# ZwwWayne/mmMOT

Hardware: AMD Instinct MI355X
Metric: frame-pairs/sec (fusion+affinity fwd) at N_det=64; affinity L∞ vs CPU ref (higher is better)
Workload: dtype f16x3

## Files before the change

include/mmmot_hip.h:

```cpp
#ifndef MMMOT_HIP_H
#define MMMOT_HIP_H

#include <stddef.h>
#include <stdint.h>

#ifdef __cplusplus
extern "C" {
#endif

#define MMMOT_OK 0
#define MMMOT_EINVAL (-1)

#define MMMOT_ACT_NONE 0
#define MMMOT_ACT_RELU 1
#define MMMOT_ACT_SIGMOID 2

#define MMMOT_A_PLAIN 0
#define MMMOT_A_NORM_RELU 1
#define MMMOT_A_PAIR 2

#define MMMOT_PAIR_MULTIPLY 0
#define MMMOT_PAIR_MINUS_ABS 1
#define MMMOT_PAIR_MINUS 2

// ... 101 lines not shown

int mmmot_gn_finalize(const float* part, const int* grp_tile0, const int* grp_ntiles,
                      const int* grp_count, const int* tile_nrows, int G, int ldp, int C, int NG,
                      const float* gamma, const float* beta, float eps,
                      float* sc, float* sh, void* stream);

int mmmot_segment_mean(const float* X, int ldx, int C,
                       const int* seg_start, const int* seg_count, const int* seg_stride,
                       const int* seg_group, const int* seg_div, int nseg,
                       const float* sc, const float* sh, int ldsc, int relu,
                       float* out, int ldo,
                       int hl16 ,
                       void* stream);

int mmmot_rowdot(const float* X, int ldx, int K, const float* w, float b,
                 const float* sc, const float* sh, int ldsc,
                 const int* tile_row0, const int* tile_nrows, const int* tile_group, int T,
                 int act, int use_thr, float thr,
                 float* out, const int* omap, void* stream);

int mmmot_row_layernorm(const float* X, int ldx, int C, const float* gamma, const float* beta,
                        float eps, int relu, float* Y, int ldy, int R, void* stream);

int mmmot_skippool_head(const float* P, int ldp, int C, int C4, const float* g0, const float* b0, const float* w1,
                        const float* c1, const float* g2, const float* b2, const float* w4, const float* c4,
                        const float* g5, const float* b5, float eps, float* out, int ldo, int R, void* stream);
int mmmot_pointnet_layer1(const float* X, int K, const float* W, const float* bias,
                          float* Y, float* part,
                          const int* tile_row0, const int* tile_nrows, int T, void* stream);

int mmmot_pn_mlp64(const float* X, int ldx, const float* sc, const float* sh, int ldsc, const void* W16,
                   float oscale, const float* bias, float* Y, int ldy, float* part, const int* tile_row0,
                   const int* tile_nrows, const int* tile_group, int T, int N, void* stream);

int mmmot_affine_act(const float* X, int ldx, int C, const float* sc, const float* sh, int ldsc,
                     const int* tile_row0, const int* tile_nrows, const int* tile_group, int T,
                     int act, float* Y, int ldy, void* stream);

int mmmot_fusion_combine(int mode, const float* cat, const float* Y0, int ld0,
                         const float* Y1, int ld1,
                         const float* sc0, const float* sh0, const float* sc1, const float* sh1, int ldsc,
                         const int* tile_row0, const int* tile_nrows, const int* tile_group, int T,
                         float* F, int Lt, int C, void* stream);

int mmmot_softmax_pairs(const float* logits, float* out,
                        const int* grp_row0, const int* grp_N, const int* grp_M, int G,
                        int max_nm ,
                        int mode, void* stream);

int mmmot_points_count(const float* pts, int P, int F, const double* planes, int NB, int pad_empty,
                       int* cnt, int* split, void* stream);
int mmmot_points_scatter(const float* pts, int P, int F, const double* planes, int NB, const int* cnt,
                         const int* split, float* out, int Fo, void* stream);
int mmmot_points_count_batched(const float* pts, int F, int NS, int NPOLY, int NBLK, int cnt_total,
                               const double* planes, const int* blk_sweep, const int* blk_first,
                               const int* sweep_row0, const int* poly0, const int* filt, const int* cnt_off,
                               int pad_empty, int* cnt, int* split, void* stream);
int mmmot_points_scatter_batched(const float* pts, int F, int NS, int NPOLY, int NBLK, int cnt_total,
                                 const double* planes, const int* blk_sweep, const int* blk_first,
                                 const int* sweep_row0, const int* poly0, const int* filt, const int* cnt_off,
                                 const int* cnt, const int* split, float* out, int Fo, void* stream);

#define MMMOT_ALIGN_MAX_CHAIN 4
#define MMMOT_ALIGN_REC 80
int mmmot_align_points(const float* pts, int F, int Q, int NS, const int* seg_row0, const double* xf, int chain,
                       float* out, long out_row0, int ldo, void* stream);
// ... 148 lines not shown
```

mmmot_amd/_lib.py:

```python
import ctypes
import os
import subprocess
import threading

_HERE = os.path.dirname(os.path.abspath(__file__))
CSRC = os.path.join(_HERE, 'csrc')
LIB_PATH = os.environ.get('MMMOT_LIB_PATH', os.path.join(_HERE, 'libmmmot_hip.so'))
SOURCES = ['conv3x3.hip', 'hl16_format.hip', 'conv3x3_hl16_patch.hip', 'gemm_rows.hip', 'gemm_wide.hip',
           'gemm_ares.hip', 'gemm_wres.hip', 'gemm_wreg.hip', 'pn_mlp64.hip', 'gram.hip', 'points_gather.hip', 'crop_resize.hip', 'crop_augment.hip','small_kernels.hip', 'backward.hip', 'train.hip', 'train_vgg.hip', 'gemm_tn_f16.hip',
           'assign.hip', 'assign_chain.hip', 'track_ids.hip', 'clear_mot.hip', 'align_points.hip', 'labels.hip', 'adam_step.hip', 'dropout.hip']
HIPCC = os.environ.get('HIPCC', '/opt/rocm/bin/hipcc')
HIPFLAGS = ['--offload-arch=gfx950', '-O3', '-std=c++17', '-fPIC']

_lock = threading.Lock()
_lib = None

c_f = ctypes.c_void_p
c_i = ctypes.c_int


class GemmArgs(ctypes.Structure):
    _fields_ = [
        ('X', c_f), ('ldx', c_i),
        ('W', c_f),
# ... 54 lines not shown
    'mmmot_gram_rows': [c_f, c_i, c_i, c_f, c_f, c_i, c_f, c_f, c_f, c_i, c_f, c_f, c_f],
    'mmmot_set_gram128_variant': [c_i],
    'mmmot_gn_finalize_gram': [c_f, c_f, c_f, c_f, c_f, c_i, c_i, c_f, c_f, c_i, c_f, c_f, ctypes.c_float, c_f, c_f, c_f, c_f],
    'mmmot_gn_finalize_gram_dbias': [c_f, c_f, c_f, c_f, c_f, c_i, c_f, c_f, c_i, c_f, c_f, c_i, c_i, c_f, c_f, ctypes.c_float,
                                     c_f, c_f, c_f, c_f],
    'mmmot_gn_finalize': [c_f, c_f, c_f, c_f, c_f, c_i, c_i, c_i, c_i, c_f, c_f, ctypes.c_float, c_f, c_f, c_f],
    'mmmot_segment_mean': [c_f, c_i, c_i, c_f, c_f, c_f, c_f, c_f, c_i, c_f, c_f, c_i, c_i, c_f, c_i, c_i, c_f],
    'mmmot_conv3x3_bn_relu_hl16_patch': [c_f, c_f, c_f, c_f, c_i, c_i, c_i, c_i, c_i, c_i, c_f, c_f],
    'mmmot_conv1_fused_hl16': [c_f, c_f, c_f, ctypes.c_float, c_f, c_f, c_f, c_f, c_i, c_i, c_i, c_f],
    'mmmot_conv3x3_bn_relu_hq8': [c_f, c_f, c_f, c_f, c_i, c_i, c_i, c_i, c_i, c_i, c_f, c_f],
    'mmmot_conv1_fused_u8': [c_f, ctypes.c_float, ctypes.c_float, ctypes.c_float, ctypes.c_float, ctypes.c_float,
                             ctypes.c_float, c_f, c_f, ctypes.c_float, c_f, c_f, c_f, c_f, c_i, c_i, c_i, c_i, c_f],
    'mmmot_u8_normalize': [c_f, c_i, c_i, c_f, c_f, c_f],
    'mmmot_conv1_fused_hq8': [c_f, c_f, c_f, ctypes.c_float, c_f, c_f, c_f, c_f, c_i, c_i, c_i, c_f],
    'mmmot_conv3x3_first_hl16': [c_f, c_f, c_f, c_f, c_i, c_i, c_i, c_i, c_f],
    'mmmot_set_patch_grid_limit': [c_i],
    'mmmot_set_patch_min_block': [c_i],
    'mmmot_trunk_range_read': [ctypes.POINTER(ctypes.c_uint), c_i],
    'mmmot_trunk_range_bind': [c_f],
    'mmmot_hl16_pack': [c_f, c_f, ctypes.c_long, c_f],
    'mmmot_hl16_unpack': [c_f, c_f, ctypes.c_long, c_f],
    'mmmot_hl16_pack_pow2': [c_f, c_f, ctypes.c_long, c_f, c_i, c_f],
    'mmmot_pow2_oscale': [c_f, c_i, c_f, c_i, c_f, c_i, c_f],
    'mmmot_conv3x3_raw_hl16': [c_f, c_f, c_f, c_f, c_i, c_i, c_i, c_i, c_i, c_f, c_f],
    'mmmot_hq8_pack': [c_f, c_f, ctypes.c_long, c_f],
    'mmmot_hq8_unpack': [c_f, c_f, ctypes.c_long, c_f],
    'mmmot_rowdot': [c_f, c_i, c_i, c_f, ctypes.c_float, c_f, c_f, c_i, c_f, c_f, c_f, c_i, c_i, c_i,
                     ctypes.c_float, c_f, c_f, c_f],
    'mmmot_row_layernorm': [c_f, c_i, c_i, c_f, c_f, ctypes.c_float, c_i, c_f, c_i, c_i, c_f],
    'mmmot_skippool_head': [c_f, c_i, c_i, c_i, c_f, c_f, c_f, c_f, c_f, c_f, c_f, c_f, c_f, c_f, ctypes.c_float, c_f, c_i, c_i,
                            c_f],
    'mmmot_pointnet_layer1': [c_f, c_i, c_f, c_f, c_f, c_f, c_f, c_f, c_i, c_f],
    'mmmot_pn_mlp64': [c_f, c_i, c_f, c_f, c_i, c_f, ctypes.c_float, c_f, c_f, c_i, c_f, c_f, c_f, c_f, c_i, c_i, c_f],
    'mmmot_affine_act': [c_f, c_i, c_i, c_f, c_f, c_i, c_f, c_f, c_f, c_i, c_i, c_f, c_i, c_f],
    'mmmot_fusion_combine': [c_i, c_f, c_f, c_i, c_f, c_i, c_f, c_f, c_f, c_f, c_i, c_f, c_f, c_f, c_i, c_f,
                             c_i, c_i, c_f],
    'mmmot_softmax_pairs': [c_f, c_f, c_f, c_f, c_f, c_i, c_i, c_i, c_f],
    'mmmot_points_count': [c_f, c_i, c_i, c_f, c_i, c_i, c_f, c_f, c_f],
    'mmmot_points_scatter': [c_f, c_i, c_i, c_f, c_i, c_f, c_f, c_f, c_i, c_f],
    'mmmot_crop_resize_norm': [c_f, c_i, c_i, c_f, c_i, c_i, c_i, c_f, c_f, c_f, c_f, c_f],
    'mmmot_crop_augment': [c_f, c_f, c_i, c_i, c_f, c_f, c_f, c_f],
    'mmmot_points_count_batched': [c_f, c_i, c_i, c_i, c_i, c_i, c_f, c_f, c_f, c_f, c_f, c_f, c_f, c_i, c_f, c_f, c_f],
    'mmmot_points_scatter_batched': [c_f, c_i, c_i, c_i, c_i, c_i, c_f, c_f, c_f, c_f, c_f, c_f, c_f, c_f, c_f, c_f, c_i, c_f],
    'mmmot_align_points': [c_f, c_i, c_i, c_i, c_f, c_f, c_i, c_f, ctypes.c_long, c_i, c_f],
    'mmmot_selftest_mfma': [c_f, c_f, c_f, c_i, c_f],
    'mmmot_gn_bwd_partial': [c_f, c_i, c_f, c_i, c_i, c_f, c_f, c_i, c_f, c_f, c_i, c_f, c_f, c_f, c_i, c_f, c_f],
    'mmmot_gn_bwd_finalize': [c_f, c_f, c_i, c_i, c_i, c_f, c_f, c_f],
    'mmmot_gn_bwd_apply': [c_f, c_i, c_f, c_i, c_i, c_f, c_f, c_i, c_f, c_f, c_i, c_f, c_f, c_f, c_f, c_i, c_f, c_i, c_f],
    'mmmot_gemm_tn': [ctypes.POINTER(GemmTnArgs), c_f],
    'mmmot_gemm_tn_f16': [ctypes.POINTER(GemmTnArgs), c_f, c_f],
    'mmmot_absmax': [c_f, c_i, ctypes.c_long, c_i, c_f, c_f],
    'mmmot_pair_bwd': [c_f, c_i, c_f, c_i, c_f, c_i, c_i, c_f, c_f, c_f, c_f, c_f, c_f, c_f, c_i, c_i, c_i, c_f],
    'mmmot_pair_expand_bwd': [c_f, c_i, c_f, c_i, c_i, c_f, c_f, c_f, c_i, c_f, c_f, c_f, c_f, c_f],
    'mmmot_segment_argmax': [c_f, c_i, c_i, c_f, c_f, c_f, c_f, c_i, c_f, c_f, c_i, c_i, c_f, c_i, c_f],
    'mmmot_pair_expand_max_bwd': [c_f, c_i, c_f, c_i, c_f, c_i, c_i, c_f, c_f, c_f, c_i, c_f, c_f, c_f, c_f, c_f],
    'mmmot_rowdot_bwd': [c_f, c_i, c_i, c_f, ctypes.c_float, c_f, c_f, c_i, c_f, c_f, c_f, c_i, c_i, c_f, c_f, c_f, c_i,
                         c_f, c_i, c_f],
    'mmmot_softmax_pairs_bwd': [c_f, c_f, c_f, c_f, c_f, c_f, c_i, c_i, c_i, c_f],
    'mmmot_fusion_c_bwd': [c_f, c_f, c_i, c_f, c_i, c_f, c_f, c_f, c_f, c_i, c_f, c_f, c_f, c_i, c_f, c_f, c_i, c_f, c_f, c_i, c_f],
    'mmmot_add_rows': [c_f, c_i, c_f, c_i, c_f, c_i, ctypes.c_long, c_i, c_f],
    'mmmot_conv3x3_raw': [c_f, c_f, c_f, c_f, c_i, c_i, c_i, c_i, c_i, c_i, c_f],
    'mmmot_rows_stats': [c_f, c_i, c_i, c_f, c_f, c_i, c_f, c_f],
    'mmmot_bn_relu_pool': [c_f, c_i, c_f, c_f, c_i, c_i, c_i, c_i, c_f, c_f],
    'mmmot_maxpool_bwd': [c_f, c_i, c_f, c_f, c_f, c_i, c_i, c_i, c_f, c_f],
    'mmmot_conv3x3_wgrad': [c_f, c_f, c_i, c_i, c_i, c_i, c_i, c_i, c_f, c_f],
    'mmmot_conv3x3_wgrad_f16': [c_f, c_f, c_i, c_i, c_i, c_i, c_i, c_i, c_f, c_f, c_f],
# ... 93 lines not shown
```

mmmot_amd/csrc/pn_mlp64.hip:

```cpp
#include "common.h"

#define PM_K 64
#define PM_LDT 72

template <int NOUT>
__global__ __launch_bounds__(256) void pn_mlp64_kernel(const float* __restrict__ X, int ldx,
                                                       const float* __restrict__ sc, const float* __restrict__ sh,
                                                       int ldsc, const u32x4* __restrict__ W16, float oscale,
                                                       const float* __restrict__ bias, float* __restrict__ Y, int ldy,
                                                       float* __restrict__ part, const int* __restrict__ tile_row0,
                                                       const int* __restrict__ tile_nrows,
                                                       const int* __restrict__ tile_group, int T) {
  constexpr int NT = NOUT / 32;
  __shared__ __attribute__((aligned(16))) _Float16 Wh[NOUT * PM_LDT];
  __shared__ __attribute__((aligned(16))) _Float16 Wl[NOUT * PM_LDT];
  __shared__ __attribute__((aligned(16))) _Float16 Ah[MM_BM * PM_LDT];
  __shared__ __attribute__((aligned(16))) _Float16 Al[MM_BM * PM_LDT];
  __shared__ float red[2][4][NOUT];
  const int tid = threadIdx.x, lane = tid & 63, wave = tid >> 6;
  const int lr = lane & 31, kh = (lane >> 5) * 8;

  for (int idx = tid; idx < NOUT * 8; idx += 256) {
    const int n = idx >> 3, u = idx & 7;
    const u32x4 hi = W16[(long)idx * 2], lo = W16[(long)idx * 2 + 1];
// ... 77 lines not shown
          s1 += acc[nt][e];
          Y[(long)(row0 + wave * 32 + mm_acc_row(e, lane)) * ldy + nt * 32 + lr] = acc[nt][e];
        }
      }
      s1 = mm_xor32_sum(s1);
      if (lane < 32) red[0][wave][nt * 32 + lr] = s1;
    }
    __syncthreads();
    const float inv = 1.f / (float)nrows;
#pragma unroll
    for (int nt = 0; nt < NT; ++nt) {
      const int n = nt * 32 + lr;
      const float tot = red[0][0][n] + red[0][1][n] + red[0][2][n] + red[0][3][n];
      const float mu = tot * inv;
      float s2 = 0.f;
#pragma unroll
      for (int e = 0; e < 16; ++e) {
        const float d = acc[nt][e] - mu;
        if (valid[e]) s2 = fmaf(d, d, s2);
      }
      s2 = mm_xor32_sum(s2);
      if (lane < 32) red[1][wave][n] = s2;
      if (wave == 0 && lane < 32) part[((long)t * 2 + 0) * NOUT + n] = tot;
    }
    __syncthreads();
    if (wave == 0 && lane < 32) {
#pragma unroll
      for (int nt = 0; nt < NT; ++nt) {
        const int n = nt * 32 + lr;
        part[((long)t * 2 + 1) * NOUT + n] = red[1][0][n] + red[1][1][n] + red[1][2][n] + red[1][3][n];
      }
    }
  }
}

extern "C" int mmmot_pn_mlp64(const float* X, int ldx, const float* sc, const float* sh, int ldsc, const void* W16,
                              float oscale, const float* bias, float* Y, int ldy, float* part, const int* tile_row0,
                              const int* tile_nrows, const int* tile_group, int T, int N, void* stream) {
  if (!X || !sc || !sh || !W16 || !Y || !part || !tile_row0 || !tile_nrows || T <= 0) return MMMOT_EINVAL;
  if ((N != 64 && N != 128) || ldx % 4 != 0 || ldsc % 4 != 0 || ldy < N) return MMMOT_EINVAL;
  if (!mm_al16(X) || !mm_al16(sc) || !mm_al16(sh) || !mm_al16(W16)) return MMMOT_EINVAL;
  const int n_cu = mm_num_cu();
  if (n_cu <= 0) return MMMOT_EINVAL;
  const int grid = T < 2 * n_cu ? T : 2 * n_cu;
  hipStream_t s = (hipStream_t)stream;
  if (N == 64)
    hipLaunchKernelGGL(pn_mlp64_kernel<64>, dim3(grid), dim3(256), 0, s, X, ldx, sc, sh, ldsc, (const u32x4*)W16, oscale,
                       bias, Y, ldy, part, tile_row0, tile_nrows, tile_group, T);
  else
    hipLaunchKernelGGL(pn_mlp64_kernel<128>, dim3(grid), dim3(256), 0, s, X, ldx, sc, sh, ldsc, (const u32x4*)W16, oscale,
                       bias, Y, ldy, part, tile_row0, tile_nrows, tile_group, T);
  return mm_check(hipGetLastError());
}
```

mmmot_amd/engine.py:

```python
import contextlib
import itertools
import os
import threading

import numpy as np
import torch

from .ops import (ACT_NONE, ACT_RELU, ACT_SIGMOID, A_NORM_RELU, A_PAIR, A_PLAIN, FUSION_MODES, PAIR_OPS,
                  SOFTMAX_MODES)
from .range_guard import RangeGuard
from .tape import norm_layer

POOL_INPUT = {'f32': 0, 'hl16': 1, 'hq8': 2}
EPS = 1e-5
_SERIALS = itertools.count(1)


def check_crop_side(S):
    if S < 32 or S % 2 != 0:
        raise ValueError('crop side %d is not supported: the HIP VGG trunk needs an even side >= 32; resize the crops '
                         '(mmmot_amd.crops.crop_resize_normalize)' % S)


def check_crop_layout(dets):
# ... 2 lines not shown
            raise ValueError('uint8 crops must be [L,S,S,3] (HWC, the output of mmmot_amd.crops.crop_resize_u8), got %s'
                             % (tuple(dets.shape),))
        S = int(dets.shape[1])
    else:
        S = int(dets.shape[-1])
    check_crop_side(S)
    return S


class Engine:
    eps = EPS

    def __init__(self, packed, ops, fusion='A', affinity_op='multiply', softmax_mode='none',
                 neg_threshold=0.0, score_arch='branch_cls', end_mode='avg', trunk=None):
        trunk = trunk or os.environ.get('MMMOT_TRUNK', 'f16x3')
        if trunk not in ('f16x3', 'f16q8', 'f32'):
            raise ValueError("trunk must be 'f16x3' (fp16 matrix cores, 3-term split), 'f16q8' (fp16 main term + "
                             "fp8 correction terms, include/mmmot_hip.h hq8) or 'f32' (exact fp32 MFMA)")
        self.trunk = trunk
        self.serial = next(_SERIALS)
        self.trunk_requested = trunk
        self.guard = RangeGuard(self)
        self.range_events = []
        self.last_out_of_range_forward = None
        self.out_of_range_window = None
        self._busy = threading.Lock()
        self._last_stream = None
        self._head_start = None
        ql = os.environ.get('MMMOT_Q8_LAYERS', '4,5,6,7,8,9,10,11,12')
        self.q8_layers = None if ql == 'all' else set(int(v) for v in ql.split(',') if v)
        self.pn_fused = os.environ.get('MMMOT_PN_FUSED', '1') != '0'
        self.pn_gram = os.environ.get('MMMOT_PN_GRAM', '1') != '0'
        self.pn_mlp64 = os.environ.get('MMMOT_PN_MLP64', '1') != '0'
        self.two_streams = os.environ.get('MMMOT_TWO_STREAMS', '0') == '1'
        self.pn_beside_trunk = os.environ.get('MMMOT_PN_BESIDE_TRUNK', '1') != '0'
        self._side = {}
        self.sp_fused = os.environ.get('MMMOT_SP_FUSED', '1') != '0'
        self.fuse_conv1 = os.environ.get('MMMOT_FUSE_CONV1', '1') != '0'
        self.q8_min_crop = int(os.environ.get('MMMOT_Q8_MIN_CROP', '64'))
        self.mlp = 'f32' if trunk == 'f32' else 'f16x3'
        if affinity_op not in PAIR_OPS:
            raise ValueError('unknown affinity_op %r' % (affinity_op,))
        if softmax_mode not in SOFTMAX_MODES and softmax_mode != 'none':
            softmax_mode = 'none'
        self.end_mode = end_mode
        self.P = packed
        self.ops = ops
        self.fusion = fusion
        self.affinity_op = affinity_op
        self.softmax_mode = softmax_mode
        self.neg_threshold = float(neg_threshold)
        self.score_arch = score_arch
        self.ws = {}
        self.dev = None
        self.keep = None
        self._tape = None
        self.conv_events = None

    def buf(self, name, *shape, device=None, dtype=torch.float32):
        if self._tape is not None:
            return torch.empty(*shape, dtype=dtype, device=device if device is not None else self.dev)
        return self._arena(name, *shape, device=device, dtype=dtype)

    def _arena(self, name, *shape, device=None, dtype=torch.float32):
        n = 1
        for s in shape:
# ... 149 lines not shown
        n, H = 0, plan.S
        for cv in self.P['vgg']:
            if cv['pool']:
                H //= 2
            n += plan.Lt * H * H * cv['cout']
        return n

    def _skippool(self, plan, s, x, hw, C, cat, fmt='f32'):
        hl16 = POOL_INPUT[fmt]
        ops, Lt, hd, T = self.ops, plan.Lt, self.P['skippool'][s], plan.det_tiles
        pooled = self.buf('sp_pool', Lt, C)
        plan.crop_segments(hw).pool(ops, x, C, pooled, partial=lambda n: self.buf('sp_partial', n, C), hl16=hl16)
        if self.sp_fused and hasattr(ops, 'skippool_head'):
            ops.skippool_head(pooled, C, hd, EPS, cat[:, 128 * s:128 * (s + 1)], Lt)
            return
        ln0 = self.buf('sp_ln0', Lt, C)
        ops.row_layernorm(pooled, C, hd['g0'], hd['b0'], EPS, False, ln0, Lt)
        C4 = hd['w1'].shape[0]
        h1 = self.buf('sp_h1', Lt, C4)
        self._gemm(hd, 'w1', T, C4, C, X=ln0, bias=hd['c1'], Y=h1)
        ln1 = self.buf('sp_ln1', Lt, C4)
        ops.row_layernorm(h1, C4, hd['g2'], hd['b2'], EPS, True, ln1, Lt)
        h2 = self.buf('sp_h2', Lt, 128)
        self._gemm(hd, 'w4', T, 128, C4, X=ln1, bias=hd['c4'], Y=h2)
        ops.row_layernorm(h2, 128, hd['g5'], hd['b5'], EPS, True, cat[:, 128 * s:128 * (s + 1)], Lt)

    def pointnet(self, plan, points, cat):
        ops, pn, T, D, Pn, Lt = self.ops, self.P['pointnet'], plan.pt_tiles, plan.det_tiles, plan.P, plan.Lt
        y1 = self.buf('pn_y1', Pn, 64)
        part = self._part(T, 64)
        ops.pointnet_layer1(points, pn['w1'], pn['b1'], y1, part, T)
        sc1, sh1 = self._finalize('pn1', part, T, 64, 64, pn['g1'], pn['be1'])
        x, sc, sh = y1, sc1, sh1
        for i, (N, K) in zip((2, 3, 4), ((64, 64), (64, 64), (128, 64))):
            y = self.buf('pn_y%d' % i, Pn, N)
            part = self._part(T, N)
            if self.pn_mlp64 and self.mlp == 'f16x3' and ('w%d_h16' % i) in pn:
                ops.pn_mlp64(pn['w%d_h16' % i], pn['w%d_os' % i], T, N, x, sc, sh, pn['b%d' % i], y, part)
            else:
                self._gemm(pn, 'w%d' % i, T, N, K, X=x, bias=pn['b%d' % i], Y=y, part=part, sc=sc, sh=sh,
                           amode=A_NORM_RELU)
            sc, sh = self._finalize('pn%d' % i, part, T, N, N, pn['g%d' % i], pn['be%d' % i])
            x = y
        seg1024 = self._norm_relu_pool(plan, 'w5', '5', 128, 1024, x, sc, sh)
        self._stash('pn_seg1024', seg1024)
        dbias = self.buf('pn_dbias', Lt, 512)
        self._gemm(pn, 'wc1b', D, 512, 1024, X=seg1024, bias=pn['bc1'], Y=dbias)
        seg512 = self._norm_relu_pool(plan, 'wc1a', 'c1', 64, 512, y1, sc1, sh1, dbias=dbias)
        yc2, sc2, sh2 = self._gemm_gn(pn, 'wc2', D, 512, 512, 'pn_yc2', 'pnc2', 16, pn['gc2'], pn['bec2'], X=seg512,
                                      bias=pn['bc2'])
        ops.affine_act(yc2, 512, sc2, sh2, D, ACT_RELU, cat[:, 512:1024])

    def _norm_relu_pool(self, plan, w, s, K, N, x, sc, sh, dbias=None):
        ops, pn, T, Lt = self.ops, self.P['pointnet'], plan.pt_tiles, plan.Lt
        name, g, be = 'pn' + s, pn['g' + s], pn['be' + s]
        if dbias is None:
            ares_kw = row_kw = dict(bias=pn['b' + s])
        else:
            ares_kw, row_kw = dict(dbias=dbias, tile_dbrow=plan.tile_det), dict(dbias=dbias, rowidx=plan.row_det)
        seg = self.buf('pn_seg%d' % N, Lt, N)
        if self.pn_fused and self.mlp == 'f16x3' and (w + '_h16') in pn:
            TD, TH = plan.ptd_tiles, plan.ptd_half
            if self.pn_gram and (dbias is None or hasattr(ops, 'gn_finalize_gram_dbias')):
                GT, gram = (plan.gram_tiles, 'gram') if dbias is None else (plan.gram64_tiles, 'gram64')
                Gp, Sp = self.buf64(gram + '_G', GT.T, K * K), self.buf64(gram + '_S', GT.T, K)
                ops.gram_rows(x, K, sc, sh, GT, Gp, Sp)
                osc, osh = self.buf(name + '_sc', GT.G, N), self.buf(name + '_sh', GT.G, N)
                work = self.buf64(gram + '_work', GT.G, K * K + K)
                if dbias is None:
                    ops.gn_finalize_gram(Gp, Sp, GT, K, pn[w], pn['b' + s], N, g, be, EPS, work, osc, osh)
                else:
                    ops.gn_finalize_gram_dbias(Gp, Sp, GT, plan.gram64_tile_det, K, pn[w], dbias, N, g, be, EPS, work,
                                               osc, osh)
            else:
                part = self._part(TH, N)
                ops.gemm_ares(pn[w + '_h16'], pn[w + '_os'], TD, N, K, x, sc, sh, part=part, **ares_kw)
                osc, osh = self._finalize(name, part, TH, N, N, g, be)
            cs = self.buf('pn_colsum', TH.T, N)
            timed = self.conv_events is not None and dbias is None
            if timed:
                e0, e1 = torch.cuda.Event(enable_timing=True), torch.cuda.Event(enable_timing=True)
                e0.record()
            ops.gemm_ares(pn[w + '_h16'], pn[w + '_os'], TD, N, K, x, sc, sh, osc=osc, osh=osh, colsum=cs, **ares_kw)
            if timed:
                e1.record()
                self.conv_events.append((name, plan.P, K, N, e0, e1))
            ops.segment_mean(cs, N, plan.det_half_segs, seg)
        elif self.pn_fused:
            TD = plan.ptd_tiles
            part = self._part(TD, N)
            self._gemm(pn, w, TD, N, K, X=x, part=part, sc=sc, sh=sh, amode=A_NORM_RELU, **row_kw)
            osc, osh = self._finalize(name, part, TD, N, N, g, be)
            cs = self.buf('pn_colsum', TD.T, N)
            self._gemm(pn, w, TD, N, K, X=x, sc=sc, sh=sh, amode=A_NORM_RELU, osc=osc, osh=osh, colsum=cs, **row_kw)
            ops.segment_mean(cs, N, plan.det_tile_segs, seg)
        else:
            y, osc, osh = self._gemm_gn(pn, w, T, N, K, 'pn_y' + s, name, N, g, be, X=x, sc=sc, sh=sh, amode=A_NORM_RELU,
                                        **row_kw)
            ops.segment_mean(y, N, plan.det_segs, seg, sc=osc, sh=osh, relu=True)
# ... 242 lines not shown
```

mmmot_amd/ops.py:

```python
import contextlib
import ctypes
import os
import threading

import torch

from . import _lib

ACT_NONE, ACT_RELU, ACT_SIGMOID = 0, 1, 2
A_PLAIN, A_NORM_RELU, A_PAIR = 0, 1, 2
PAIR_OPS = {'multiply': 0, 'minus_abs': 1, 'minus': 2}
SOFTMAX_MODES = {'single': 1, 'dual': 2, 'dual_add': 3, 'dual_max': 4}
FUSION_MODES = {'A': 0, 'B': 1, 'C': 2}
LOSS_KINDS = {'bce': 0, 'l2': 1, 'l1': 2}


def _ptr(t, dtype=torch.float32):
    if t is None:
        return None
    if not t.is_cuda:
        raise RuntimeError('mmmot_amd HIP ops need device tensors (got %s); there is no CPU fallback' % t.device)
    if t.dtype != dtype:
        raise TypeError('expected %s, got %s' % (dtype, t.dtype))
    return t.data_ptr()
# ... 176 lines not shown
        a.FA, a.FB, a.ldf = _ptr(FA), _ptr(FB), _ld(FA)
        a.tile_row0, a.tile_nrows, a.tile_group = _iptr(tiles.row0), _iptr(tiles.nrows), _iptr(tiles.group)
        if pair is not None:
            a.grp_row0, a.grp_M = _iptr(pair['row0']), _iptr(pair['M'])
            a.grp_aoff, a.grp_boff = _iptr(pair['aoff']), _iptr(pair['boff'])
            a.pair_uniform32 = int(bool(pair.get('uniform32', False)))
        a.T, a.N, a.K = tiles.T, N, K
        a.amode, a.pairop, a.act = amode, pairop, act
        a.w_hl16, a.oscale = int(w_hl16), float(oscale)
        a.osc, a.osh, a.ldosc = _ptr(osc), _ptr(osh), _ld(osc)
        a.colsum = _ptr(colsum)
        _lib.check(self.lib.mmmot_gemm_rows(ctypes.byref(a), self._stream()), 'mmmot_gemm_rows')

    def gemm_ares(self, W16, oscale, tiles, N, K, X, sc, sh, bias=None, dbias=None, tile_dbrow=None, part=None,
                  osc=None, osh=None, colsum=None):
        a = _lib.GemmAresArgs()
        a.X, a.ldx = _ptr(X), _ld(X)
        a.sc, a.sh, a.ldsc = _ptr(sc), _ptr(sh), _ld(sc)
        a.W, a.bias = _ptr(W16), _ptr(bias)
        a.dbias, a.tile_dbrow, a.lddb = _ptr(dbias), _iptr(tile_dbrow), _ld(dbias)
        a.tile_row0, a.tile_nrows, a.tile_group = _iptr(tiles.row0), _iptr(tiles.nrows), _iptr(tiles.group)
        a.part = _ptr(part)
        a.osc, a.osh, a.ldosc = _ptr(osc), _ptr(osh), _ld(osc)
        a.colsum = _ptr(colsum)
        a.T, a.N, a.K, a.oscale = tiles.T, N, K, float(oscale)
        _lib.check(self.lib.mmmot_gemm_ares(ctypes.byref(a), self._stream()), 'mmmot_gemm_ares')

    def pn_mlp64(self, W16, oscale, tiles, N, X, sc, sh, bias, Y, part):
        st = self.lib.mmmot_pn_mlp64(_ptr(X), _ld(X), _ptr(sc), _ptr(sh), _ld(sc), _ptr(W16), float(oscale),
                                     _ptr(bias), _ptr(Y), _ld(Y), _ptr(part), _iptr(tiles.row0), _iptr(tiles.nrows),
                                     _iptr(tiles.group), tiles.T, N, self._stream())
        _lib.check(st, 'mmmot_pn_mlp64')

    def gram_rows(self, X, K, sc, sh, tiles, Gout, Sout):
        st = self.lib.mmmot_gram_rows(_ptr(X), _ld(X), K, _ptr(sc), _ptr(sh), _ld(sc), _iptr(tiles.row0),
                                      _iptr(tiles.nrows), _iptr(tiles.group), tiles.T,
                                      _ptr(Gout, torch.float64), _ptr(Sout, torch.float64), self._stream())
        _lib.check(st, 'mmmot_gram_rows')

    def gn_finalize_gram(self, Gp, Sp, tiles, K, W, bias, N, gamma, beta, eps, work, sc, sh):
        st = self.lib.mmmot_gn_finalize_gram(_ptr(Gp, torch.float64), _ptr(Sp, torch.float64), _iptr(tiles.g_tile0),
                                             _iptr(tiles.g_ntiles), _iptr(tiles.g_count), tiles.G, K, _ptr(W),
                                             _ptr(bias), N, _ptr(gamma), _ptr(beta), float(eps),
                                             _ptr(work, torch.float64), _ptr(sc), _ptr(sh), self._stream())
        _lib.check(st, 'mmmot_gn_finalize_gram')

    def gn_finalize_gram_dbias(self, Gp, Sp, tiles, tile_det, K, W, dbias, N, gamma, beta, eps, work, sc, sh):
        st = self.lib.mmmot_gn_finalize_gram_dbias(_ptr(Gp, torch.float64), _ptr(Sp, torch.float64), _iptr(tiles.g_tile0),
                                                   _iptr(tiles.g_ntiles), _iptr(tiles.g_count), tiles.G, _iptr(tiles.nrows),
                                                   _iptr(tile_det), K, _ptr(W), _ptr(dbias), _ld(dbias), N, _ptr(gamma),
                                                   _ptr(beta), float(eps), _ptr(work, torch.float64), _ptr(sc), _ptr(sh),
                                                   self._stream())
        _lib.check(st, 'mmmot_gn_finalize_gram_dbias')

    def gn_finalize(self, part, tiles, C, NG, gamma, beta, eps, sc, sh):
        if part.dim() != 3 or part.stride(2) != 1 or part.stride(0) != 2 * part.stride(1):
            raise ValueError('part must be a [T][2][C] view of a [T][2][ldp] buffer')
        st = self.lib.mmmot_gn_finalize(_ptr(part), _iptr(tiles.g_tile0), _iptr(tiles.g_ntiles),
                                        _iptr(tiles.g_count), _iptr(tiles.nrows) if tiles.ragged else None, tiles.G,
                                        part.stride(1), C, NG, _ptr(gamma), _ptr(beta),
                                        float(eps), _ptr(sc), _ptr(sh), self._stream())
        _lib.check(st, 'mmmot_gn_finalize')

    def segment_mean(self, X, C, segs, out, sc=None, sh=None, relu=False, use_group=True, hl16=False, take_max=False):
        st = self.lib.mmmot_segment_mean(_ptr(X), _ld(X), C, _iptr(segs.start), _iptr(segs.count),
                                         _iptr(segs.stride), _iptr(segs.group) if use_group else None,
# ... 270 lines not shown
```

mmmot_amd/profiler.py:

```python
import time

import torch

PEAK_F16X3_TFLOPS = 2500.0 / 3.0
PEAK_F32_TFLOPS = 157.3
PEAK_HBM_TBS = 8.0


def _rows(t):
    return int(getattr(t, 'R', 0))


def _seg_rows(segs):
    return int(segs.h_count.sum())


def _conv(name):
    def cost(a, k):
        inp, wp, bias, out, L, H, W, Cin, Cout = a[:9]
        pool = a[10] if name == 'conv3x3' else a[9]
        Ho, Wo = (H // 2, W // 2) if pool else (H, W)
        fl = 2.0 * L * H * W * 9 * Cin * Cout
        by = 4.0 * (L * H * W * Cin + L * Ho * Wo * Cout + 9 * Cin * Cout)
        return ('trunk conv %d->%d @%dx%d%s' % (Cin, Cout, H, W, ' +pool' if pool else ''), fl, by)
# ... 3 lines not shown
def _conv1_fused(a, k):
    i = max(j for j, v in enumerate(a) if torch.is_tensor(v))
    L, H, W = a[i + 1:i + 4]
    fl = 2.0 * L * H * W * 9 * (3 * 64 + 64 * 64)
    by = (1.0 if a[0].dtype == torch.uint8 else 4.0) * L * H * W * 3 + 4.0 * L * (H // 2) * (W // 2) * 64
    return ('trunk conv1_1+conv1_2 (fused) 3->64->64 @%dx%d +pool' % (H, W), fl, by)


def _gemm(a, k):
    W, tiles, N, K = a[:4]
    R = _rows(tiles)
    amode = k.get('amode', 0)
    kind = {0: 'plain', 1: 'norm+relu prologue', 2: 'pair prologue'}[amode]
    by = 4.0 * N * K + (4.0 * R * N if k.get('Y') is not None else 0.0)
    if amode != 2 and k.get('X') is not None:
        by += 4.0 * R * K
    if k.get('colsum') is not None or (k.get('Y') is None and k.get('part') is not None):
        kind += ', reduced'
    big = 'rows GEMM' if R >= 4096 else 'small GEMM'
    return ('%s %d->%d (%s)' % (big, K, N, kind), 2.0 * R * N * K, by)


def _gemm_ares(a, k):
    W16, oscale, tiles, N, K, X = a[:6]
    R = _rows(tiles)
    what = 'column sums' if k.get('colsum') is not None else 'statistics'
    return ('A-resident GEMM %d->%d (norm+relu prologue, %s only)' % (K, N, what), 2.0 * R * N * K, 4.0 * R * K + 4.0 * N * K)


def _pn_mlp64(a, k):
    W16, oscale, tiles, N = a[:4]
    R = _rows(tiles)
    return ('PointNet layer 64->%d (pn_mlp64)' % N, 2.0 * R * 64 * N, 4.0 * R * (64 + N))


def _gram(a, k):
    X, K, sc, sh, tiles = a[:5]
    R = _rows(tiles)
    return ('Gram matrix of the %d-channel rows (conv5 statistics)' % K, 2.0 * R * K * K, 4.0 * R * K)


def _segment_mean(a, k):
    X, C, segs, out = a[:4]
    R = _seg_rows(segs)
    kind = 'hl16 rows' if k.get('hl16') else ('norm+relu rows' if k.get('sc') is not None else 'rows')
    big = 'segment mean' if R >= 65536 else 'small segment mean'
    return ('%s, %d channels (%s)' % (big, C, kind), 1.0 * R * C, 4.0 * R * C)


def _rowdot(a, k):
    X, K, w, b, tiles, out = a[:6]
    R = _rows(tiles)
    return ('row dot %d->1' % K, 2.0 * R * K, 4.0 * R * K)


def _latency(label):
    return lambda a, k: (label, 0.0, 0.0)


def _layer1(a, k):
    X, W, bias, Y, part, tiles = a[:6]
    R = _rows(tiles)
    Kin = int(W.shape[1])
    return ('PointNet layer %d->64 (points in)' % Kin, 2.0 * R * Kin * 64, 4.0 * R * (Kin + 64))


COSTS = {
    'conv3x3': _conv('conv3x3'),
    'conv3x3_hl16_patch': _conv('hl16'),
    'conv3x3_hq8': _conv('hq8'),
    'conv1_fused_hl16': _conv1_fused,
    'conv1_fused_hq8': _conv1_fused,
    'conv1_fused_u8': _conv1_fused,
    'conv3x3_first_hl16': lambda a, k: ('trunk conv1_1 3->%d (fp32 MFMA)' % a[7], 2.0 * a[4] * a[5] * a[6] * 27 * a[7],
                                        4.0 * a[4] * a[5] * a[6] * (3 + a[7])),
    'gemm': _gemm,
    'gemm_ares': _gemm_ares,
    'pn_mlp64': _pn_mlp64,
    'gram_rows': _gram,
    'gn_finalize_gram': _latency('GroupNorm scale/shift from the Gram matrix'),
    'gn_finalize_gram_dbias': _latency('GroupNorm scale/shift from the Gram matrix'),
    'gn_finalize': _latency('GroupNorm scale/shift from tile partials'),
    'segment_mean': _segment_mean,
    'rowdot': _rowdot,
    'row_layernorm': _latency('row LayerNorm'),
    'skippool_head': _latency('SkipPool head (LN, 1x1, LN, 1x1, LN)'),
    'pointnet_layer1': _layer1,
    'affine_act': _latency('affine + activation rows'),
    'fusion_combine': _latency('fusion combine'),
    'softmax_pairs': _latency('pair softmax'),
    'u8_normalize': _latency('8-bit crops -> fp32'),
    'crop_augment': lambda a, k: ('augmented 8-bit crops -> fp32', 0.0,
                                  1.0 * a[5] * a[6] * a[6] * (3 + (12 if a[3] is not None else 0) + (3 if a[4] is not None else 0))),
    'hq8_pack': _latency('hq8 / hl16 re-encode'), 'hq8_unpack': _latency('hq8 / hl16 re-encode'),
    'hl16_pack': _latency('hq8 / hl16 re-encode'), 'hl16_unpack': _latency('hq8 / hl16 re-encode'),
}


class LaunchProfiler:

    def __init__(self, ops, f32=False):
        self.ops = ops
        self.cuda = torch.cuda.is_available()
        self.peak_tf = PEAK_F32_TFLOPS if f32 else PEAK_F16X3_TFLOPS
        self.records = []
        self._saved = {}

    def _wrap(self, name, fn, cost):
        def wrapped(*a, **k):
            try:
                label, fl, by = cost(a, k)
# ... 76 lines not shown
```

Before: 305.4.

## Fuse PointNet layers 2 and 3 into one kernel using Gram-derived GroupNorm stats

Adds a kernel that runs PointNet layers 2 and 3 back to back in one pass. Layer-2 GroupNorm scale/shift are computed beforehand from the Gram matrix of the normalized layer-1 output, so layer 2's output never goes to global memory and no stats pass is needed between the layers. The Gram result is reused for the wc1a norm/pool path, so it is no longer computed twice. This removes one launch, one stats finalize, and a round trip of the intermediate activations, at the cost of more LDS per block and extra eligibility checks.

Result: no change. 306.7 (median of 6 runs) (+0.4%).

```diff
diff --git a/include/mmmot_hip.h b/include/mmmot_hip.h
--- a/include/mmmot_hip.h
+++ b/include/mmmot_hip.h
@@ -157,6 +157,11 @@
 int mmmot_pn_mlp64(const float* X, int ldx, const float* sc, const float* sh, int ldsc, const void* W16,
                    float oscale, const float* bias, float* Y, int ldy, float* part, const int* tile_row0,
                    const int* tile_nrows, const int* tile_group, int T, int N, void* stream);
+
+int mmmot_pn_mlp64x2(const float* X, int ldx, const float* sc1, const float* sh1, int ldsc1, const void* W2,
+                     float oscale2, const float* bias2, const float* sc2, const float* sh2, int ldsc2, const void* W3,
+                     float oscale3, const float* bias3, float* Y, int ldy, float* part, const int* tile_row0,
+                     const int* tile_nrows, const int* tile_group, int T, void* stream);
 
 int mmmot_affine_act(const float* X, int ldx, int C, const float* sc, const float* sh, int ldsc,
                      const int* tile_row0, const int* tile_nrows, const int* tile_group, int T,
diff --git a/mmmot_amd/_lib.py b/mmmot_amd/_lib.py
--- a/mmmot_amd/_lib.py
+++ b/mmmot_amd/_lib.py
@@ -110,6 +110,8 @@
                             c_f],
     'mmmot_pointnet_layer1': [c_f, c_i, c_f, c_f, c_f, c_f, c_f, c_f, c_i, c_f],
     'mmmot_pn_mlp64': [c_f, c_i, c_f, c_f, c_i, c_f, ctypes.c_float, c_f, c_f, c_i, c_f, c_f, c_f, c_f, c_i, c_i, c_f],
+    'mmmot_pn_mlp64x2': [c_f, c_i, c_f, c_f, c_i, c_f, ctypes.c_float, c_f, c_f, c_f, c_i, c_f, ctypes.c_float, c_f, c_f, c_i,
+                         c_f, c_f, c_f, c_f, c_i, c_f],
     'mmmot_affine_act': [c_f, c_i, c_i, c_f, c_f, c_i, c_f, c_f, c_f, c_i, c_i, c_f, c_i, c_f],
     'mmmot_fusion_combine': [c_i, c_f, c_f, c_i, c_f, c_i, c_f, c_f, c_f, c_f, c_i, c_f, c_f, c_f, c_i, c_f,
                              c_i, c_i, c_f],
diff --git a/mmmot_amd/csrc/pn_mlp64.hip b/mmmot_amd/csrc/pn_mlp64.hip
--- a/mmmot_amd/csrc/pn_mlp64.hip
+++ b/mmmot_amd/csrc/pn_mlp64.hip
@@ -133,6 +133,188 @@
       }
     }
   }
+}
+
+__global__ __launch_bounds__(256) void pn_mlp64x2_kernel(
+    const float* __restrict__ X, int ldx, const float* __restrict__ sc1, const float* __restrict__ sh1, int ldsc1,
+    const u32x4* __restrict__ W2, float oscale2, const float* __restrict__ bias2, const float* __restrict__ sc2,
+    const float* __restrict__ sh2, int ldsc2, const u32x4* __restrict__ W3, float oscale3,
+    const float* __restrict__ bias3, float* __restrict__ Y, int ldy, float* __restrict__ part,
+    const int* __restrict__ tile_row0, const int* __restrict__ tile_nrows, const int* __restrict__ tile_group, int T) {
+  constexpr int NOUT = 64, NT = 2;
+  __shared__ __attribute__((aligned(16))) _Float16 Wh[2][NOUT * PM_LDT];
+  __shared__ __attribute__((aligned(16))) _Float16 Wl[2][NOUT * PM_LDT];
+  __shared__ __attribute__((aligned(16))) _Float16 Ah[MM_BM * PM_LDT];
+  __shared__ __attribute__((aligned(16))) _Float16 Al[MM_BM * PM_LDT];
+  __shared__ float red[2][4][NOUT];
+  const int tid = threadIdx.x, lane = tid & 63, wave = tid >> 6;
+  const int lr = lane & 31, kh = (lane >> 5) * 8;
+
+  for (int idx = tid; idx < 2 * NOUT * 8; idx += 256) {
+    const int l = idx >> 9, i = idx & 511, n = i >> 3, u = i & 7;
+    const u32x4* W16 = l ? W3 : W2;
+    const u32x4 hi = W16[(long)i * 2], lo = W16[(long)i * 2 + 1];
+    *reinterpret_cast<u32x4*>(&Wh[l][n * PM_LDT + u * 8]) = hi;
+    *reinterpret_cast<u32x4*>(&Wl[l][n * PM_LDT + u * 8]) = lo;
+  }
+  const int srow = tid >> 4, sc0 = (tid & 15) * 4;
+  f32x4 x[8];
+  auto load_rows = [&](int tt) {
+    const int row0 = tile_row0[tt], nrows = tile_nrows[tt];
+#pragma unroll
+    for (int i = 0; i < 8; ++i) {
+      const int r = srow + 16 * i;
+      x[i] = *reinterpret_cast<const f32x4*>(X + (long)(row0 + (r < nrows ? r : 0)) * ldx + sc0);
+    }
+  };
+  int t = blockIdx.x;
+  if (t < T) load_rows(t);
+  float bv2[NT], bv3[NT];
+#pragma unroll
+  for (int nt = 0; nt < NT; ++nt) {
+    bv2[nt] = bias2 ? bias2[nt * 32 + lr] : 0.f;
+    bv3[nt] = bias3 ? bias3[nt * 32 + lr] : 0.f;
+  }
+  const int offa = (wave * 32 + lr) * PM_LDT + kh;
+  auto layer = [&](const _Float16* wh, const _Float16* wl, f32x16 (&acc)[NT]) {
+#pragma unroll
+    for (int nt = 0; nt < NT; ++nt)
+#pragma unroll
+      for (int e = 0; e < 16; ++e) acc[nt][e] = 0.f;
+#pragma unroll
+    for (int j = 0; j < PM_K / 16; ++j) {
+      const f16x8 ah = *reinterpret_cast<const f16x8*>(&Ah[offa + j * 16]);
+      const f16x8 al = *reinterpret_cast<const f16x8*>(&Al[offa + j * 16]);
+#pragma unroll
+      for (int nt = 0; nt < NT; ++nt) {
+        const int offb = (nt * 32 + lr) * PM_LDT + kh + j * 16;
+        const f16x8 bh = *reinterpret_cast<const f16x8*>(&wh[offb]);
+        const f16x8 bl = *reinterpret_cast<const f16x8*>(&wl[offb]);
+        acc[nt] = __builtin_amdgcn_mfma_f32_32x32x16_f16(al, bh, acc[nt], 0, 0, 0);
+        acc[nt] = __builtin_amdgcn_mfma_f32_32x32x16_f16(ah, bl, acc[nt], 0, 0, 0);
+        acc[nt] = __builtin_amdgcn_mfma_f32_32x32x16_f16(ah, bh, acc[nt], 0, 0, 0);
+      }
+    }
+  };
+
+  for (; t < T; t += gridDim.x) {
+    const int row0 = tile_row0[t], nrows = tile_nrows[t];
+    const int grp = tile_group ? tile_group[t] : 0;
+    {
+      const f32x4 s0 = *reinterpret_cast<const f32x4*>(sc1 + (long)grp * ldsc1 + sc0);
+      const f32x4 h0 = *reinterpret_cast<const f32x4*>(sh1 + (long)grp * ldsc1 + sc0);
+#pragma unroll
+      for (int i = 0; i < 8; ++i) {
+        const int r = srow + 16 * i;
+        float y[4];
+#pragma unroll
+        for (int e = 0; e < 4; ++e) {
+          y[e] = mm_norm_relu(x[i][e], s0[e], h0[e]);
+          if (r >= nrows) y[e] = 0.f;
+        }
+        unsigned h0_, l0_, h1_, l1_;
+        mm_split2(y[0], y[1], h0_, l0_);
+        mm_split2(y[2], y[3], h1_, l1_);
+        *reinterpret_cast<u32x2*>(&Ah[r * PM_LDT + sc0]) = u32x2{h0_, h1_};
+        *reinterpret_cast<u32x2*>(&Al[r * PM_LDT + sc0]) = u32x2{l0_, l1_};
+      }
+    }
+    const int tn = t + gridDim.x;
+    if (tn < T) load_rows(tn);
+    float s2v[NT], h2v[NT];
+#pragma unroll
+    for (int nt = 0; nt < NT; ++nt) {
+      s2v[nt] = sc2[(long)grp * ldsc2 + nt * 32 + lr];
+      h2v[nt] = sh2[(long)grp * ldsc2 + nt * 32 + lr];
+    }
+    __syncthreads();
+    bool valid[16];
+#pragma unroll
+    for (int e = 0; e < 16; ++e) valid[e] = wave * 32 + mm_acc_row(e, lane) < nrows;
+    f32x16 acc[NT];
+    layer(Wh[0], Wl[0], acc);
+#pragma unroll
+    for (int nt = 0; nt < NT; ++nt)
+#pragma unroll
+      for (int e = 0; e < 16; e += 2) {
+        float y[2];
+#pragma unroll
+        for (int q = 0; q < 2; ++q) {
+          y[q] = mm_norm_relu(fmaf(acc[nt][e + q], oscale2, bv2[nt]), s2v[nt], h2v[nt]);
+          if (!valid[e + q]) y[q] = 0.f;
+        }
+        unsigned h_, l_;
+        mm_split2(y[0], y[1], h_, l_);
+        const f16x2 hh = __builtin_bit_cast(f16x2, h_), ll = __builtin_bit_cast(f16x2, l_);
+#pragma unroll
+        for (int q = 0; q < 2; ++q) {
+          const int o = (wave * 32 + mm_acc_row(e + q, lane)) * PM_LDT + nt * 32 + lr;
+          Ah[o] = hh[q];
+          Al[o] = ll[q];
+        }
+      }
+    __builtin_amdgcn_fence(__ATOMIC_RELEASE, "wavefront");
+    __builtin_amdgcn_wave_barrier();
+    __builtin_amdgcn_fence(__ATOMIC_ACQUIRE, "wavefront");
+    layer(Wh[1], Wl[1], acc);
+#pragma unroll
+    for (int nt = 0; nt < NT; ++nt) {
+      float s1 = 0.f;
+#pragma unroll
+      for (int e = 0; e < 16; ++e) {
+        acc[nt][e] = fmaf(acc[nt][e], oscale3, bv3[nt]);
+        if (valid[e]) {
+          s1 += acc[nt][e];
+          Y[(long)(row0 + wave * 32 + mm_acc_row(e, lane)) * ldy + nt * 32 + lr] = acc[nt][e];
+        }
+      }
+      s1 = mm_xor32_sum(s1);
+      if (lane < 32) red[0][wave][nt * 32 + lr] = s1;
+    }
+    __syncthreads();
+    const float inv = 1.f / (float)nrows;
+#pragma unroll
+    for (int nt = 0; nt < NT; ++nt) {
+      const int n = nt * 32 + lr;
+      const float tot = red[0][0][n] + red[0][1][n] + red[0][2][n] + red[0][3][n];
+      const float mu = tot * inv;
+      float s2 = 0.f;
+#pragma unroll
+      for (int e = 0; e < 16; ++e) {
+        const float d = acc[nt][e] - mu;
+        if (valid[e]) s2 = fmaf(d, d, s2);
+      }
+      s2 = mm_xor32_sum(s2);
+      if (lane < 32) red[1][wave][n] = s2;
+      if (wave == 0 && lane < 32) part[((long)t * 2 + 0) * NOUT + n] = tot;
+    }
+    __syncthreads();
+    if (wave == 0 && lane < 32) {
+#pragma unroll
+      for (int nt = 0; nt < NT; ++nt) {
+        const int n = nt * 32 + lr;
+        part[((long)t * 2 + 1) * NOUT + n] = red[1][0][n] + red[1][1][n] + red[1][2][n] + red[1][3][n];
+      }
+    }
+  }
+}
+
+extern "C" int mmmot_pn_mlp64x2(const float* X, int ldx, const float* sc1, const float* sh1, int ldsc1, const void* W2,
+                                float oscale2, const float* bias2, const float* sc2, const float* sh2, int ldsc2,
+                                const void* W3, float oscale3, const float* bias3, float* Y, int ldy, float* part,
+                                const int* tile_row0, const int* tile_nrows, const int* tile_group, int T,
+                                void* stream) {
+  if (!X || !sc1 || !sh1 || !W2 || !sc2 || !sh2 || !W3 || !Y || !part || !tile_row0 || !tile_nrows || T <= 0)
+    return MMMOT_EINVAL;
+  if (ldx % 4 != 0 || ldsc1 % 4 != 0 || ldsc2 < 64 || ldy < 64) return MMMOT_EINVAL;
+  if (!mm_al16(X) || !mm_al16(sc1) || !mm_al16(sh1) || !mm_al16(W2) || !mm_al16(W3)) return MMMOT_EINVAL;
+  const int n_cu = mm_num_cu();
+  if (n_cu <= 0) return MMMOT_EINVAL;
+  const int grid = T < 2 * n_cu ? T : 2 * n_cu;
+  hipLaunchKernelGGL(pn_mlp64x2_kernel, dim3(grid), dim3(256), 0, (hipStream_t)stream, X, ldx, sc1, sh1, ldsc1,
+                     (const u32x4*)W2, oscale2, bias2, sc2, sh2, ldsc2, (const u32x4*)W3, oscale3, bias3, Y, ldy, part,
+                     tile_row0, tile_nrows, tile_group, T);
+  return mm_check(hipGetLastError());
 }
 
 extern "C" int mmmot_pn_mlp64(const float* X, int ldx, const float* sc, const float* sh, int ldsc, const void* W16,
diff --git a/mmmot_amd/engine.py b/mmmot_amd/engine.py
--- a/mmmot_amd/engine.py
+++ b/mmmot_amd/engine.py
@@ -58,6 +58,7 @@
         self.pn_fused = os.environ.get('MMMOT_PN_FUSED', '1') != '0'
         self.pn_gram = os.environ.get('MMMOT_PN_GRAM', '1') != '0'
         self.pn_mlp64 = os.environ.get('MMMOT_PN_MLP64', '1') != '0'
+        self.pn_fuse23 = os.environ.get('MMMOT_PN_FUSE23', '1') != '0'
         self.two_streams = os.environ.get('MMMOT_TWO_STREAMS', '0') == '1'
         self.pn_beside_trunk = os.environ.get('MMMOT_PN_BESIDE_TRUNK', '1') != '0'
         self._side = {}
@@ -273,7 +274,22 @@
         ops.pointnet_layer1(points, pn['w1'], pn['b1'], y1, part, T)
         sc1, sh1 = self._finalize('pn1', part, T, 64, 64, pn['g1'], pn['be1'])
         x, sc, sh = y1, sc1, sh1
-        for i, (N, K) in zip((2, 3, 4), ((64, 64), (64, 64), (128, 64))):
+        layers, gram64 = ((2, 64, 64), (3, 64, 64), (4, 128, 64)), None
+        if self._pn_fuse23(plan):
+            GT = plan.gram64_tiles
+            gram64 = self.buf64('gram64_G', GT.T, 64 * 64), self.buf64('gram64_S', GT.T, 64)
+            ops.gram_rows(y1, 64, sc1, sh1, GT, *gram64)
+            sc2, sh2 = self.buf('pn2_sc', GT.G, 64), self.buf('pn2_sh', GT.G, 64)
+            work = self.buf64('gram64_work', GT.G, 64 * 64 + 64)
+            ops.gn_finalize_gram(gram64[0], gram64[1], GT, 64, pn['w2'], pn['b2'], 64, pn['g2'], pn['be2'], EPS, work,
+                                 sc2, sh2)
+            x = self.buf('pn_y3', Pn, 64)
+            part = self._part(T, 64)
+            ops.pn_mlp64x2(pn['w2_h16'], pn['w2_os'], pn['b2'], pn['w3_h16'], pn['w3_os'], pn['b3'], T, y1, sc1, sh1,
+                           sc2, sh2, x, part)
+            sc, sh = self._finalize('pn3', part, T, 64, 64, pn['g3'], pn['be3'])
+            layers = layers[2:]
+        for i, N, K in layers:
             y = self.buf('pn_y%d' % i, Pn, N)
             part = self._part(T, N)
             if self.pn_mlp64 and self.mlp == 'f16x3' and ('w%d_h16' % i) in pn:
@@ -287,12 +303,19 @@
         self._stash('pn_seg1024', seg1024)
         dbias = self.buf('pn_dbias', Lt, 512)
         self._gemm(pn, 'wc1b', D, 512, 1024, X=seg1024, bias=pn['bc1'], Y=dbias)
-        seg512 = self._norm_relu_pool(plan, 'wc1a', 'c1', 64, 512, y1, sc1, sh1, dbias=dbias)
+        seg512 = self._norm_relu_pool(plan, 'wc1a', 'c1', 64, 512, y1, sc1, sh1, dbias=dbias, gram_done=gram64)
         yc2, sc2, sh2 = self._gemm_gn(pn, 'wc2', D, 512, 512, 'pn_yc2', 'pnc2', 16, pn['gc2'], pn['bec2'], X=seg512,
                                       bias=pn['bc2'])
         ops.affine_act(yc2, 512, sc2, sh2, D, ACT_RELU, cat[:, 512:1024])
 
-    def _norm_relu_pool(self, plan, w, s, K, N, x, sc, sh, dbias=None):
+    def _pn_fuse23(self, plan):
+        ops, pn = self.ops, self.P['pointnet']
+        return (self.pn_fuse23 and self.pn_mlp64 and self.pn_fused and self.pn_gram and self.mlp == 'f16x3'
+                and self._tape is None and all(k in pn for k in ('w2_h16', 'w3_h16', 'wc1a_h16'))
+                and hasattr(ops, 'pn_mlp64x2') and hasattr(ops, 'gn_finalize_gram_dbias')
+                and np.array_equal(plan.gram64_tiles.h_g_count, plan.pt_tiles.h_g_count))
+
+    def _norm_relu_pool(self, plan, w, s, K, N, x, sc, sh, dbias=None, gram_done=None):
         ops, pn, T, Lt = self.ops, self.P['pointnet'], plan.pt_tiles, plan.Lt
         name, g, be = 'pn' + s, pn['g' + s], pn['be' + s]
         if dbias is None:
@@ -304,8 +327,11 @@
             TD, TH = plan.ptd_tiles, plan.ptd_half
             if self.pn_gram and (dbias is None or hasattr(ops, 'gn_finalize_gram_dbias')):
                 GT, gram = (plan.gram_tiles, 'gram') if dbias is None else (plan.gram64_tiles, 'gram64')
-                Gp, Sp = self.buf64(gram + '_G', GT.T, K * K), self.buf64(gram + '_S', GT.T, K)
-                ops.gram_rows(x, K, sc, sh, GT, Gp, Sp)
+                if gram_done is None:
+                    Gp, Sp = self.buf64(gram + '_G', GT.T, K * K), self.buf64(gram + '_S', GT.T, K)
+                    ops.gram_rows(x, K, sc, sh, GT, Gp, Sp)
+                else:
+                    Gp, Sp = gram_done
                 osc, osh = self.buf(name + '_sc', GT.G, N), self.buf(name + '_sh', GT.G, N)
                 work = self.buf64(gram + '_work', GT.G, K * K + K)
                 if dbias is None:
diff --git a/mmmot_amd/ops.py b/mmmot_amd/ops.py
--- a/mmmot_amd/ops.py
+++ b/mmmot_amd/ops.py
@@ -232,6 +232,13 @@
                                      _iptr(tiles.group), tiles.T, N, self._stream())
         _lib.check(st, 'mmmot_pn_mlp64')
 
+    def pn_mlp64x2(self, W2, oscale2, bias2, W3, oscale3, bias3, tiles, X, sc1, sh1, sc2, sh2, Y, part):
+        st = self.lib.mmmot_pn_mlp64x2(_ptr(X), _ld(X), _ptr(sc1), _ptr(sh1), _ld(sc1), _ptr(W2), float(oscale2),
+                                       _ptr(bias2), _ptr(sc2), _ptr(sh2), _ld(sc2), _ptr(W3), float(oscale3),
+                                       _ptr(bias3), _ptr(Y), _ld(Y), _ptr(part), _iptr(tiles.row0), _iptr(tiles.nrows),
+                                       _iptr(tiles.group), tiles.T, self._stream())
+        _lib.check(st, 'mmmot_pn_mlp64x2')
+
     def gram_rows(self, X, K, sc, sh, tiles, Gout, Sout):
         st = self.lib.mmmot_gram_rows(_ptr(X), _ld(X), K, _ptr(sc), _ptr(sh), _ld(sc), _iptr(tiles.row0),
                                       _iptr(tiles.nrows), _iptr(tiles.group), tiles.T,
diff --git a/mmmot_amd/profiler.py b/mmmot_amd/profiler.py
--- a/mmmot_amd/profiler.py
+++ b/mmmot_amd/profiler.py
@@ -59,6 +59,11 @@
     W16, oscale, tiles, N = a[:4]
     R = _rows(tiles)
     return ('PointNet layer 64->%d (pn_mlp64)' % N, 2.0 * R * 64 * N, 4.0 * R * (64 + N))
+
+
+def _pn_mlp64x2(a, k):
+    R = _rows(a[6])
+    return ('PointNet layers 64->64->64 in one pass (pn_mlp64x2)', 2.0 * 2 * R * 64 * 64, 4.0 * R * (64 + 64))
 
 
 def _gram(a, k):
@@ -104,6 +109,7 @@
     'gemm': _gemm,
     'gemm_ares': _gemm_ares,
     'pn_mlp64': _pn_mlp64,
+    'pn_mlp64x2': _pn_mlp64x2,
     'gram_rows': _gram,
     'gn_finalize_gram': _latency('GroupNorm scale/shift from the Gram matrix'),
     'gn_finalize_gram_dbias': _latency('GroupNorm scale/shift from the Gram matrix'),
```
